# KudanLimited/cuda-bundle-adjustment

Measured on AMD Instinct MI355X. Metric: ba_edge_iterations_per_sec, higher is better.
Workload: dtype f64

## Files before the change

cuda-bundle-adjustment_amd/csrc/host/c_api.cpp:

```cpp
#include <cmath>
#include <cstring>
#include <deque>
#include <memory>
#include <unordered_map>

#include "../../../include/cugo_hip.h"
#include "../../include/cuda_graph_optimisation.h"
#include "../../include/icp_types.h"
#include "../kernels/kernels.h"
#include "chol_solver.h"
#include "engine.h"
#include "hip_util.h"
#include "rccl_comm.h"
#include "schur_plan.h"

using namespace cugo_host;

namespace
{
template <typename F>
int guarded(F&& f)
{
    try
    {
// ... 349 lines not shown
    return CUGO_OK;
}

int cugo_chol_plan_array(cugo_chol* s, const char* name, const int32_t** out)
{
    const CholPlan& P = s->plan;
    const std::string n(name);
    const std::vector<int32_t>* v = nullptr;
#define CUGO_PLAN_FIELD(f) \
    if (n == #f)           \
    v = &P.f
    CUGO_PLAN_FIELD(perm);
    CUGO_PLAN_FIELD(super_ptr);
    CUGO_PLAN_FIELD(rows_ptr);
    CUGO_PLAN_FIELD(rows);
    CUGO_PLAN_FIELD(sparent);
    CUGO_PLAN_FIELD(child_ptr);
    CUGO_PLAN_FIELD(child);
    CUGO_PLAN_FIELD(rel_ptr);
    CUGO_PLAN_FIELD(rel);
    CUGO_PLAN_FIELD(ncb);
    CUGO_PLAN_FIELD(nb);
    CUGO_PLAN_FIELD(col0);
    CUGO_PLAN_FIELD(col_front);
    CUGO_PLAN_FIELD(stage_task_ptr);
    CUGO_PLAN_FIELD(task_ptr);
    CUGO_PLAN_FIELD(task_fronts);
    CUGO_PLAN_FIELD(blk_front);
    CUGO_PLAN_FIELD(blk_row);
    CUGO_PLAN_FIELD(blk_col);
    CUGO_PLAN_FIELD(alias_of);
    CUGO_PLAN_FIELD(asm_map);
    CUGO_PLAN_FIELD(wl);
#undef CUGO_PLAN_FIELD
    if (n == "asm_info")
    {
        s->asm_info.assign(1, P.asm0);
        s->asm_info.push_back(P.nasm);
        for (int64_t o : P.asm_off)
            s->asm_info.push_back((int32_t)o);
        v = &s->asm_info;
    }
    if (n == "blk_trans")
        v = &s->trans32;
    if (n == "ea1")
        v = &s->ea1;
    if (!v)
    {
        set_last_error("cugo_chol_plan_array: unknown array " + n);
        return CUGO_ERR_INVALID;
    }
    *out = v->data();
    return (int)v->size();
}

int cugo_chol_plan_array64(cugo_chol* s, const char* name, const int64_t** out)
{
    const CholPlan& P = s->plan;
    const std::string n(name);
    const std::vector<int64_t>* v = n == "off" ? &P.off : n == "ldf" ? &P.ldf : n == "woff" ? &P.woff
                                  : n == "l21off" ? &P.l21off : nullptr;
    if (!v)
    {
        set_last_error("cugo_chol_plan_array64: unknown array " + n);
        return CUGO_ERR_INVALID;
    }
// ... 552 lines not shown
```

cuda-bundle-adjustment_amd/csrc/host/chol_solver.cpp:

```cpp
#include "chol_solver.h"

#include <cstdio>
#include <cstdlib>
#include <cstring>
#include <string>

using namespace cugo_host;

void cugo_chol::pack()
{
    const CholPlan& P = plan;
    pack32.clear(), pack64.clear();
    auto put32 = [this](const std::vector<int32_t>& v) {
        const size_t o = pack32.size();
        pack32.insert(pack32.end(), v.begin(), v.end());
        pack32.resize((pack32.size() + 3) & ~size_t(3));
        return o;
    };
    auto put64 = [this](const std::vector<int64_t>& v) {
        const size_t o = pack64.size();
        pack64.insert(pack64.end(), v.begin(), v.end());
        pack64.resize((pack64.size() + 1) & ~size_t(1));
        return o;
    };
// ... 53 lines not shown
        const int64_t q[4] = {P.off[f], P.ldf[f], P.woff[f], P.l21off[f]};
        std::memcpy(m + 8, q, sizeof q);
    }
    const size_t o_tmeta = put32(tmeta);
    std::vector<int32_t> fat(16 * (P.wl.size() / 3), 0);
    for (size_t i = 0; i < P.wl.size() / 3; i++)
    {
        int32_t* m = fat.data() + 16 * i;
        const int f = P.wl[3 * i];
        m[0] = f, m[1] = P.wl[3 * i + 1], m[2] = P.wl[3 * i + 2];
        if (f < 0 || f >= P.n_super)
            continue;
        m[3] = 6 * P.ncb[f], m[4] = 6 * (P.nb[f] - P.ncb[f]);
        m[5] = P.bw_np[f], m[6] = P.col0[f], m[7] = P.rows_ptr[f];
        const int64_t q[4] = {P.off[f], P.ldf[f], P.woff[f], P.l21off[f]};
        std::memcpy(m + 8, q, sizeof q);
        if ((int)i >= P.asm0 && (int)i < P.asm0 + P.nasm)
        {
            const int64_t nb = P.nb[f], mo = P.asm_off[f];
            m[5] = (int32_t)nb;
            std::memcpy(m + 6, &mo, sizeof mo);
            bool any = false;
            for (int64_t cb = m[1]; cb < m[2]; cb++)
            {
                any = any || P.asm_map[mo + cb] >= 0;
                const int64_t c0 = mo + nb + cb * nb - cb * (cb - 1) / 2;
                for (int64_t k = 0; k < nb - cb && !any; k++)
                    any = P.asm_map[c0 + k] >= 0;
            }
            m[4] = any ? 1 : 0;
        }
    }
    const size_t o_fat = put32(fat);
    const size_t o_asm_map = put32(P.asm_map);
    const size_t o_trans = pack32.size();
    pack32.resize(o_trans + (P.blk_trans.size() + 3) / 4 + 4, 0);
    if (!P.blk_trans.empty())
        std::memcpy(pack32.data() + o_trans, P.blk_trans.data(), P.blk_trans.size());
    const size_t o_asm_off = put64(P.asm_off);
    const size_t o_off = put64(P.off), o_woff = put64(P.woff), o_l21off = put64(P.l21off), o_ldf = put64(P.ldf);
    po = {o_ncb, o_nb, o_col0, o_alias, o_bwnp, o_lanp, o_rows_ptr, o_rows, o_child_ptr, o_child, o_rel_ptr, o_rel,
          o_task_ptr, o_task_fronts, o_blk_front, o_blk_row, o_blk_col, o_perm, o_col_front, o_wl, o_ea1, o_tmeta,
          o_fat, o_asm_map, o_trans, o_asm_off, o_off, o_woff, o_l21off, o_ldf};
}

void cugo_chol::upload(hipStream_t s)
{
    const CholPlan& P = plan;
    const size_t o_ncb = po[0], o_nb = po[1], o_col0 = po[2], o_alias = po[3], o_bwnp = po[4], o_lanp = po[5];
    const size_t o_rows_ptr = po[6], o_rows = po[7], o_child_ptr = po[8], o_child = po[9], o_rel_ptr = po[10];
    const size_t o_rel = po[11], o_task_ptr = po[12], o_task_fronts = po[13], o_blk_front = po[14], o_blk_row = po[15];
    const size_t o_blk_col = po[16], o_perm = po[17], o_col_front = po[18], o_wl = po[19], o_ea1 = po[20];
    const size_t o_tmeta = po[21], o_fat = po[22], o_asm_map = po[23], o_trans = po[24], o_asm_off = po[25];
    const size_t o_off = po[26], o_woff = po[27], o_l21off = po[28], o_ldf = po[29];
    d_pack32.upload(pack32, s), d_pack64.upload(pack64, s);
    d_fronts.resize((size_t)P.front_doubles + 16);
    d_fronts.zero(s);
    d_xnew.resize((size_t)6 * P.n + 16);
    d_junk.resize(64 * 1024);
    d_winv.resize((size_t)P.winv_doubles + 16);
    d_l21.resize((size_t)P.l21_doubles + 16);
    CUGO_HIP(hipStreamSynchronize(s));

    cugo_k::CholPlanDev& D = dev;
    D.n_fronts = P.n_super;
    const int32_t* b32 = d_pack32.data();
    const int64_t* b64 = d_pack64.data();
    D.ncb = b32 + o_ncb, D.nb = b32 + o_nb, D.off = b64 + o_off, D.col0 = b32 + o_col0;
    D.rows_ptr = b32 + o_rows_ptr, D.rows = b32 + o_rows;
    D.child_ptr = b32 + o_child_ptr, D.child = b32 + o_child;
    D.rel_ptr = b32 + o_rel_ptr, D.rel = b32 + o_rel;
    D.n_stages = P.n_stages;
    D.task_ptr = b32 + o_task_ptr, D.task_fronts = b32 + o_task_fronts, D.tmeta = b32 + o_tmeta;
    D.n_hsc_blocks = (int)P.blk_front.size();
    D.blk_front = b32 + o_blk_front, D.blk_row = b32 + o_blk_row;
    D.blk_col = b32 + o_blk_col, D.blk_trans = reinterpret_cast<const uint8_t*>(b32 + o_trans);
    D.n = P.n, D.perm = b32 + o_perm, D.col_front = b32 + o_col_front;
    D.junk = d_junk.data();
    D.woff = b64 + o_woff, D.winv = d_winv.data(), D.nc_max = P.nc_max;
    D.ea_lds = opt.ea_lds, D.panel16 = opt.panel16, D.ea_direct = opt.ea_direct;
#ifdef CUGO_DEBUG_HOOKS
    {
        const char* ka = std::getenv("CUGO_KERNEL_ACQUIRE");
        D.kernel_acquire = ka ? std::atoi(ka) & 7 : 0;
        const char* ed = std::getenv("CUGO_DEBUG_DELAY");
        D.dbg_delay = ed ? std::atoi(ed) : 0;
        const char* ez = std::getenv("CUGO_DEBUG_ZERO_LDS");
        D.zero_lds = ez ? std::atoi(ez) : 0, D.lds_doubles = 0;
        D.dbg_skip_wg = -1;
    }
#endif
    D.l21off = b64 + o_l21off, D.l21 = d_l21.data();
    D.ldf = b64 + o_ldf, D.alias_of = b32 + o_alias, D.bw_np = b32 + o_bwnp, D.la_np = b32 + o_lanp;
    d_wl_ptr = b32 + o_wl;
    D.wl_base = d_wl_ptr, D.fat = b32 + o_fat, D.ea1 = b32 + o_ea1;
    D.asm_map = b32 + o_asm_map, D.asm_off = b64 + o_asm_off;
    asm_fronts = opt.asm_fronts;
    lds_factor = cugo_k::chol_lds_factor_bytes(P.nc_max);
    lds_backward = cugo_k::chol_lds_backward_bytes(P.nc_max, P.ld_max);
}

void cugo_chol::analyze(int n, const int32_t* rowptr, const int32_t* colind)
{
    analyze_host(n, rowptr, colind);
    if (ctx)
        upload(ctx->stream);
}

void cugo_chol::analyze_host(int n, const int32_t* rowptr, const int32_t* colind)
{
    CholOptions copt = CholOptions::from_env();
    const bool own_forced = opt.own_subtrees == 1;
    if ((world > 1 || own_forced) && bcast && opt.own_subtrees != 0)
        copt.rank = rank, copt.world = world, copt.owned = true;
    chol_analyze(n, rowptr, colind, copt, plan);
    if (copt.owned && !own_forced && plan.flops < 1e9 * opt.own_min_gflop)
    {
        copt.rank = 0, copt.world = 1, copt.owned = false;
        chol_analyze(n, rowptr, colind, copt, plan);
    }
    lookahead = opt.lookahead;
    factored = false, si_ready = false, last_fail = nullptr;
    trans32.assign(plan.blk_trans.begin(), plan.blk_trans.end());
    pack();
    if (plan.nc_max > cugo_k::chol_max_pivot_cols() ||
        cugo_k::chol_lds_factor_bytes(plan.nc_max) > 160 * 1024 ||
        cugo_k::chol_lds_backward_bytes(plan.nc_max, plan.ld_max) > 160 * 1024)
        throw std::runtime_error("cugo: a front exceeds the LDS budget (nc=" +
                                 std::to_string(plan.nc_max) + ", ld=" + std::to_string(plan.ld_max) + ")");
// ... 143 lines not shown
    void keep_arrays(double* d_x)
    {
        if (!keep_on || c.dbg_calls > 16)
            return;
        const cugo_host::CholPlan& plan = c.plan;
        const size_t nf = (size_t)plan.front_doubles, nw = (size_t)plan.winv_doubles, nl = (size_t)plan.l21_doubles,
                     nx = (size_t)6 * plan.n;
        while (c.keep.size() < (size_t)c.dbg_calls)
            c.keep.emplace_back(new cugo_host::DevBuf<double>());
        auto& k = *c.keep[c.dbg_calls - 1];
        k.resize(nf + nw + nl + 2 * nx + 8);
        double* dst = k.data();
        const std::pair<const double*, size_t> parts[] = {{c.d_fronts.data(), nf}, {c.d_winv.data(), nw}, {c.d_l21.data(), nl},
                                                          {c.d_xnew.data(), nx}, {d_x, nx}};
        for (const auto& pr : parts)
        {
            if (pr.second)
                CUGO_HIP(hipMemcpyAsync(dst, pr.first, pr.second * sizeof(double), hipMemcpyDeviceToDevice, s));
            dst += pr.second;
        }
        g_last_kept = &c;
    }
};
#define CUGO_HOOK(expr) expr
#else
cugo_chol::~cugo_chol() {}
#define CUGO_HOOK(expr) ((void)0)
#endif

void cugo_chol::factor_solve(const double* d_Hsc, double lambda, const double* d_bsc, double* d_x,
                             int32_t* d_fail)
{
    hipStream_t s = ctx->stream;
    factored = true, last_fail = d_fail;
#ifdef CUGO_DEBUG_HOOKS
    cugo_chol_hooks hooks(*this);
#endif
#ifdef CUGO_STAMPS
    static const bool dbg = std::getenv("CUGO_DEBUG_STAMPS") != nullptr;
    static long long* d_stamps = nullptr;
    if (dbg && !d_stamps)
    {
        CUGO_HIP(hipMalloc(reinterpret_cast<void**>(&d_stamps), 64 * sizeof(long long)));
        CUGO_HIP(hipMemset(d_stamps, 0, 64 * sizeof(long long)));
        cugo_k::set_debug_stamps(d_stamps);
    }
#endif
    cugo_k::launch_chol_assemble(s, dev, d_fronts.data(), (size_t)plan.front_doubles, d_Hsc, lambda, d_bsc, d_fail,
                                 d_wl_ptr + 3L * plan.clr0, plan.nclr, asm_fronts ? d_wl_ptr + 3L * plan.asm0 : nullptr,
                                 plan.nasm);
    CUGO_HOOK(hooks.hash(11, d_fronts.data(), (size_t)plan.front_doubles));
    int pend0 = 0, npend = 0, pend_tile = 64;
    for (int st = 0; st < plan.n_stages; st++)
    {
        const int t0 = plan.stage_task_ptr[st], t1 = plan.stage_task_ptr[st + 1];
        if (plan.has_subtree_stage && st == 0)
            cugo_k::launch_chol_subtree_stage(s, dev, d_fronts.data(), t0, t1 - t0, lds_factor, d_fail);
        else if (lookahead)
        {
            cugo_k::launch_chol_potrf_la(s, dev, d_fronts.data(), t0, t1 - t0, d_wl_ptr + 3L * pend0, npend,
                                         pend_tile, d_fail);
            cugo_k::launch_chol_lead(s, dev, d_fronts.data(), d_wl_ptr + 3L * plan.lead_ptr[st],
                                     plan.lead_ptr[st + 1] - plan.lead_ptr[st], d_wl_ptr + 3L * plan.ea_ptr[st],
                                     plan.ea_ptr[st + 1] - plan.ea_ptr[st], d_wl_ptr + 3L * plan.eab_ptr[st],
                                     plan.eab_ptr[st + 1] - plan.eab_ptr[st]);
            pend0 = plan.sb_ptr[st], npend = plan.sb_ptr[st + 1] - plan.sb_ptr[st];
// ... 9 lines not shown
                plan.ea_ptr[st + 1] - plan.ea_ptr[st], plan.eab_ptr[st],
                plan.eab_ptr[st + 1] - plan.eab_ptr[st], plan.syrk_ptr[st],
                plan.syrk_ptr[st + 1] - plan.syrk_ptr[st], plan.stage_tile[st], lds_factor, d_fail, stale, stale_scratch);
            if (plan.stage_tile[st] == 0)
            {
                cugo_k::launch_chol_two_phase(s, dev, d_fronts.data(), d_wl_ptr + 3L * plan.trsm_ptr[st],
                                              plan.trsm_ptr[st + 1] - plan.trsm_ptr[st],
                                              d_wl_ptr + 3L * plan.syrk_ptr[st],
                                              plan.syrk_ptr[st + 1] - plan.syrk_ptr[st]);
                CUGO_HOOK(hooks.after_two_phase(st));
            }
        }
        CUGO_HOOK(hooks.after_level(st));
        bool grouped = false;
        for (size_t k = 0; k < plan.xu_front.size(); k++)
            if (plan.xu_stage[k] == st)
            {
                if (!grouped && bcast_group)
                    bcast_group(true), grouped = true;
                const int f = plan.xu_front[k];
                const int64_t ld = plan.ldf[f], c0 = 6LL * plan.ncb[f], c1 = 6LL * plan.nb[f];
                if (c1 > c0)
                    bcast(d_fronts.data() + plan.off[f] + c0 * ld + c0, (size_t)((c1 - 1 - c0) * ld + c1 + 1 - c0),
                          plan.xu_owner[k]);
            }
        if (grouped)
            bcast_group(false);
    }
    if (npend > 0)
        cugo_k::launch_chol_potrf_la(s, dev, d_fronts.data(), 0, 0, d_wl_ptr + 3L * pend0, npend, pend_tile, d_fail);
    CUGO_HOOK(hooks.hash(12, d_winv.data(), (size_t)plan.winv_doubles));
    CUGO_HOOK(hooks.hash(13, d_l21.data(), (size_t)plan.l21_doubles));
    CUGO_HOOK(hooks.hash(14, d_fronts.data(), (size_t)plan.front_doubles));
    for (int st = plan.n_stages - 1; st >= 0; st--)
    {
        const int t0 = plan.stage_task_ptr[st], t1 = plan.stage_task_ptr[st + 1];
        cugo_k::launch_chol_backward_stage(s, dev, d_fronts.data(), t0, t1 - t0, lds_backward, d_xnew.data(),
                                           d_x, d_wl_ptr + 3L * plan.bwg_ptr[st],
                                           plan.bwg_ptr[st + 1] - plan.bwg_ptr[st]);
        CUGO_HOOK(hooks.after_backward(st));
#ifdef CUGO_STAMPS
        if (dbg && st == plan.n_stages - 1)
        {
            CUGO_HIP(hipStreamSynchronize(s));
            CUGO_HIP(hipMemcpy(d_stamps + 48, d_stamps + 24, 8 * sizeof(long long), hipMemcpyDeviceToDevice));
        }
#endif
    }
    CUGO_HOOK(hooks.hash(15, d_xnew.data(), (size_t)6 * plan.n));
    if (!plan.xx_lo.empty())
    {
        if (bcast_group)
            bcast_group(true);
        for (size_t k = 0; k < plan.xx_lo.size(); k++)
            bcast(d_xnew.data() + 6LL * plan.xx_lo[k], (size_t)(6LL * (plan.xx_hi[k] - plan.xx_lo[k])), plan.xx_owner[k]);
        if (bcast_group)
            bcast_group(false);
        cugo_k::launch_chol_unpermute(s, dev, d_xnew.data(), d_x);
    }
    CUGO_HIP(hipGetLastError());
    CUGO_HOOK(hooks.keep_arrays(d_x));
#ifdef CUGO_STAMPS
    if (dbg)
    {
        long long h[64];
        CUGO_HIP(hipStreamSynchronize(s));
        CUGO_HIP(hipMemcpy(h, d_stamps, sizeof h, hipMemcpyDeviceToHost));
        static int calls = 0;
        if (++calls == 5)
            for (int k = 0; k < 7; k++)
            {
                std::printf("stamps kernel %d (nc=%lld):", k, h[k * 8 + 6]);
                for (int i = 1; i < 8; i++)
                    if (i != 6 && h[k * 8 + i])
                        std::printf(" [%d] +%lld", i, h[k * 8 + i] - h[k * 8]);
                std::printf("  (cycles since kernel start; last launch of the kernel)\n");
            }
    }
#endif
}

bool cugo_chol::selected_inverse(double* d_sigma)
{
    hipStream_t s = ctx->stream;
    int32_t h_fail = 0;
    CUGO_HIP(hipMemcpyAsync(&h_fail, last_fail, sizeof h_fail, hipMemcpyDeviceToHost, s));
    CUGO_HIP(hipStreamSynchronize(s));
    if (h_fail)
        return false;
    const CholPlan& P = plan;
    if (!si_ready)
    {
        std::vector<int64_t> sinfo(4 * (size_t)P.n_super + 4, 0);
        for (int f = 0; f < P.n_super; f++)
        {
            const int pa = P.sparent[f];
            if (pa < 0)
                continue;
            sinfo[4 * f] = P.off[pa], sinfo[4 * f + 1] = P.ldf[pa], sinfo[4 * f + 2] = P.rel_ptr[f];
            sinfo[4 * f + 3] = P.alias_of[pa] == f ? 0 : 1;
        }
        const int tile = cugo_k::selinv_row_tile();
        std::vector<int32_t> items;
        si_ptr.assign(P.n_stages + 1, 0);
        for (int st = 0; st < P.n_stages; st++)
        {
            si_ptr[st] = (int32_t)(items.size() / 2);
            if (!(P.has_subtree_stage && st == 0))
                for (int t = P.stage_task_ptr[st]; t < P.stage_task_ptr[st + 1]; t++)
                    for (int fi = P.task_ptr[t]; fi < P.task_ptr[t + 1]; fi++)
                    {
                        const int f = P.task_fronts[fi];
                        for (int r0 = 0; r0 < 6 * (P.nb[f] - P.ncb[f]); r0 += tile)
                            items.push_back(f), items.push_back(r0);
                    }
        }
        si_ptr[P.n_stages] = (int32_t)(items.size() / 2);
        items.resize(items.size() + 2, 0);
        d_sinfo.upload(sinfo, s);
        d_sitems.upload(items, s);
// ... 22 lines not shown
```

cuda-bundle-adjustment_amd/csrc/host/chol_solver.h:

```cpp
#pragma once
#include "../kernels/kernels.h"
#include "chol_symbolic.h"
#include "hip_util.h"
#include "options.h"

#include <array>
#include <functional>
#include <memory>

struct cugo_chol
{
    cugo_ctx* ctx = nullptr;
    bool analyzed = false;
    cugo_host::Options opt = cugo_host::Options::from_env();
    cugo_host::CholPlan plan;
    std::vector<int32_t> trans32;
    std::vector<int32_t> asm_info;
    std::vector<int32_t> ea1;
    cugo_k::CholPlanDev dev{};
    size_t lds_factor = 0, lds_backward = 0;
    bool lookahead = false;
    bool asm_fronts = true;

    std::vector<int32_t> pack32;
    std::vector<int64_t> pack64;
    std::array<size_t, 30> po{};
    cugo_host::DevBuf<int32_t> d_pack32;
    cugo_host::DevBuf<int64_t> d_pack64;
    const int32_t* d_wl_ptr = nullptr;
    cugo_host::DevBuf<double> d_fronts, d_xnew, d_junk, d_winv, d_l21;

    int rank = 0, world = 1;
    std::function<void(double*, size_t, int)> bcast;
    std::function<void(bool)> bcast_group;
    ~cugo_chol();
#ifdef CUGO_DEBUG_HOOKS
    unsigned long long* dbg_hash = nullptr;
    int dbg_calls = 0;
    std::vector<std::unique_ptr<cugo_host::DevBuf<double>>> keep;
    cugo_host::DevBuf<double> dbg_scratch;
    void dump_kept(const char* dir);
    void dump_slot(int call, const char* path);
#endif
    bool own_subtrees() const { return bcast && plan.owned; }

    const int32_t* last_fail = nullptr;
    bool factored = false;
    bool si_ready = false;
    cugo_host::DevBuf<double> d_sig;
    cugo_host::DevBuf<int64_t> d_sinfo;
    cugo_host::DevBuf<int32_t> d_sitems;
    std::vector<int32_t> si_ptr;
    bool selected_inverse(double* d_sigma);

    void analyze(int n, const int32_t* rowptr, const int32_t* colind);
    void analyze_host(int n, const int32_t* rowptr, const int32_t* colind);
    void pack();
    void upload(hipStream_t s);
    void factor_solve(const double* d_Hsc, double lambda, const double* d_bsc, double* d_x,
                      int32_t* d_fail);
};

#ifdef CUGO_DEBUG_HOOKS
// ... 5 lines not shown
```

cuda-bundle-adjustment_amd/csrc/host/chol_symbolic.cpp:

```cpp
#include "chol_symbolic.h"

#include <algorithm>
#include <atomic>
#include <chrono>
#include <cstdio>
#include <cstdlib>
#include <functional>
#include <numeric>
#include <stdexcept>
#include <thread>
#include <tuple>

namespace cugo_host
{

CholOptions CholOptions::from_env()
{
    CholOptions o;
    if (const char* s = std::getenv("CUGO_ND_LEAF"))
        o.nd_leaf = std::max(1, std::atoi(s));
    if (const char* s = std::getenv("CUGO_MAX_SUPER_COLS"))
        o.max_super_cols = std::max(1, std::atoi(s));
    if (const char* s = std::getenv("CUGO_ZERO_FRAC"))
        o.zero_frac = std::atof(s);
// ... 1420 lines not shown
                P.asm_off[f] = (int64_t)P.asm_map.size();
                P.asm_map.resize(P.asm_map.size() + nb + nb * (nb + 1) / 2, -1);
                for (int cb = 0; cb < nb; cb += 2)
                {
                    P.wl.push_back(f), P.wl.push_back(cb), P.wl.push_back((int)std::min<int64_t>(nb, cb + 2));
                    P.nasm++;
                }
            }
        for (int f = 0; f < ns; f++)
            if (P.asm_off[root[f]] >= 0)
                for (int c = 0; c < P.ncb[f]; c++)
                    P.asm_map[P.asm_off[root[f]] + shift[f] + c] = P.col0[f] + c;
        for (size_t k = 0; k < P.blk_front.size(); k++)
        {
            const int f = P.blk_front[k], o = root[f];
            if (P.asm_off[o] < 0)
                continue;
            const int64_t nb = P.nb[o], rb = P.blk_row[k] + shift[f], cb = P.blk_col[k] + shift[f];
            if (rb < cb || rb >= nb)
                throw std::runtime_error("cugo: an Hsc block outside the lower triangle of its front");
            int32_t& e = P.asm_map[P.asm_off[o] + nb + cb * nb - cb * (cb - 1) / 2 + (rb - cb)];
            if (e != -1)
                throw std::runtime_error("cugo: two Hsc blocks in one front position");
            e = 2 * (int32_t)k + (rb != cb && P.blk_trans[k] ? 1 : 0);
        }
    }
    for (auto& v : P.lead_ptr)
        v += (int)P.wl.size() / 3;
    P.wl.insert(P.wl.end(), lead.begin(), lead.end());
    for (auto& v : P.sb_ptr)
        v += (int)P.wl.size() / 3;
    P.wl.insert(P.wl.end(), sb.begin(), sb.end());
    lap("8 work items");
}

}
```

cuda-bundle-adjustment_amd/csrc/host/chol_symbolic.h:

```cpp
#pragma once
#include <cstdint>
#include <vector>

namespace cugo_host
{

struct CholOptions
{
    int nd_refine = 1;
    int nd_leaf = 96;
    int max_super_cols = 16;
    double zero_frac = 0.35;
    int target_tasks = 1024;
    bool alias_chains = true;
    int min_subtree_tasks = 1 << 30;
    int max_front_cols = 16;
    int two_phase_min_tiles = 260;
    bool xcd_affinity = true;
    int tile32_max_tiles = 64;
    int rank = 0, world = 1;
    bool owned = false;
    static CholOptions from_env();
};

// ... 7 lines not shown
    std::vector<int32_t> rows_ptr, rows;
    std::vector<int32_t> sparent;
    std::vector<int32_t> child_ptr, child;
    std::vector<int32_t> rel_ptr, rel;
    std::vector<int32_t> ncb, nb, col0;
    std::vector<int64_t> off;
    int64_t front_doubles = 0;
    std::vector<int64_t> ldf;
    std::vector<int32_t> alias_of;
    int n_aliased = 0;
    std::vector<int64_t> woff;
    int64_t winv_doubles = 0;
    std::vector<int64_t> l21off;
    int64_t l21_doubles = 0;
    std::vector<int32_t> col_front;

    int n_stages = 0;
    int sum_slots = 0;
    int nd_refined = 0;
    std::vector<int32_t> stage_task_ptr;
    std::vector<int32_t> task_ptr, task_fronts;
    bool has_subtree_stage = false;
    std::vector<int32_t> wl;
    std::vector<int32_t> ea_ptr, eab_ptr, syrk_ptr, bwg_ptr;
    int clr0 = 0, nclr = 0;
    int asm0 = 0, nasm = 0;
    std::vector<int32_t> asm_map;
    std::vector<int64_t> asm_off;
    std::vector<int32_t> la_np;
    std::vector<int32_t> lead_ptr, sb_ptr;
    std::vector<int32_t> stage_tile;
    std::vector<int32_t> trsm_ptr;
    std::vector<int32_t> bw_np;
    int nc_max = 6;

    std::vector<int32_t> owner;
    std::vector<int32_t> xu_front, xu_stage, xu_owner;
    std::vector<int32_t> xx_lo, xx_hi, xx_owner;
    double rank_flops = 0, top_flops = 0;
    bool owned = false;
    int64_t xs_seg = 0, xs_top = 0;
    std::vector<int64_t> xs_off;

    std::vector<int32_t> blk_front, blk_row, blk_col;
    std::vector<uint8_t> blk_trans;

    long ld_max = 1;
    double nnzL = 0;
    double flops = 0;
    double up_potrf_flops = 0, up_trsm_flops = 0, up_syrk_flops = 0, up_ea_bytes = 0, backward_bytes = 0;
};

void chol_analyze(int n, const int32_t* rowptr, const int32_t* colind, const CholOptions& opt,
                  CholPlan& plan);

}
```

cuda-bundle-adjustment_amd/csrc/host/options.h:

```cpp
#pragma once
#include <cstdlib>

namespace cugo_host
{

struct Options
{
    int hsc_mfma = 1;
    bool hsc_xcd = true;
    bool hsc_rows = false, hsc_strip = false, schur_plan = false;
    bool fuse_t = true;
    bool pose_schur = true;
    bool float32 = false;
    bool speculate = true, trial_event = true, trial_poll = true;
    bool trial_from_build = true;
    bool profile = false;
    bool init_timing = false;
    bool structure_reuse = true;
    bool flatten_reuse = true;
    bool async_structure = true;
    bool host_structure = false;
    bool upload_thread = true;
    int own_subtrees = -1;
    double own_min_gflop = 3.0;
    bool lookahead = false;
    bool ea_lds = true, panel16 = true, asm_fronts = true;
    bool ea_direct = true;
    bool reduce_scatter = true;

    static Options from_env()
    {
        Options o;
        auto flag = [](const char* name) { return std::getenv(name) != nullptr; };
        auto off = [](const char* name) {
            const char* e = std::getenv(name);
            return e && e[0] == '0';
        };
        auto on = [](const char* name) {
            const char* e = std::getenv(name);
            return e && e[0] == '1';
        };
        if (const char* e = std::getenv("CUGO_HSC_MFMA"))
            o.hsc_mfma = e[0] == '0' ? 0 : e[0] == '2' ? 2 : 1;
        o.hsc_xcd = !off("CUGO_HSC_XCD");
        o.schur_plan = flag("CUGO_SCHUR_PLAN");
        o.hsc_rows = on("CUGO_HSC_ROWS"), o.hsc_strip = on("CUGO_HSC_STRIP");
        o.fuse_t = !off("CUGO_FUSE_T");
        o.pose_schur = !off("CUGO_POSE_SCHUR");
        o.float32 = on("CUGO_FLOAT32");
        o.speculate = !off("CUGO_SPECULATE"), o.trial_event = !off("CUGO_TRIAL_EVENT"), o.trial_poll = !off("CUGO_TRIAL_POLL");
        o.trial_from_build = !off("CUGO_TRIAL_FROM_BUILD");
        o.profile = flag("CUGO_PROFILE");
        o.init_timing = flag("CUGO_INIT_TIMING");
        o.structure_reuse = !flag("CUGO_NO_STRUCTURE_REUSE");
        o.flatten_reuse = !flag("CUGO_NO_FLATTEN_REUSE");
        o.async_structure = !off("CUGO_ASYNC_STRUCTURE");
        o.host_structure = flag("CUGO_HOST_STRUCTURE");
        o.upload_thread = !off("CUGO_UPLOAD_THREAD");
        if (const char* e = std::getenv("CUGO_OWN_SUBTREES"))
            o.own_subtrees = e[0] == '1' ? 1 : e[0] == '0' ? 0 : -1;
        if (const char* e = std::getenv("CUGO_OWN_MIN_GFLOP"))
            o.own_min_gflop = std::atof(e);
        if (const char* e = std::getenv("CUGO_LOOKAHEAD"))
            o.lookahead = std::atoi(e) != 0;
        o.ea_lds = !off("CUGO_EA_LDS"), o.panel16 = !off("CUGO_PANEL16"), o.asm_fronts = !off("CUGO_ASM_FRONTS");
        o.ea_direct = !off("CUGO_EA_DIRECT");
        o.reduce_scatter = !off("CUGO_REDUCE_SCATTER");
        return o;
    }
};

}
```

cuda-bundle-adjustment_amd/csrc/kernels/chol_kernels.hip:

```cpp
#include <algorithm>
#include <cstdio>

#include "kernels.h"

namespace
{

constexpr int CBS = 256;
constexpr double PIVOT_TOL = 1e-14;
constexpr int TR = 64;
constexpr int NC_MAX = 96;
constexpr int LLD = NC_MAX + 17;
constexpr int PW = 6;

using cugo_k::CholPlanDev;
typedef double double4_t __attribute__((ext_vector_type(4)));

__device__ __forceinline__ void assemble_scatter(const CholPlanDev& p, double* __restrict__ fronts,
                                                 const double* __restrict__ Hsc, double lambda,
                                                 const double* __restrict__ bsc, int32_t* __restrict__ fail, int nblk,
                                                 int bid)
{
    if (bid >= nblk)
    {
// ... 2155 lines not shown

__global__ __launch_bounds__(BIG) void k_backward_stage(CholPlanDev p,
                                                        const double* __restrict__ fronts,
                                                        int task0, int ntasks,
                                                        const int32_t* __restrict__ wl_gemv,
                                                        double* __restrict__ xnew,
                                                        double* __restrict__ xout)
{
#ifdef CUGO_DEBUG_HOOKS
    if (p.dbg_skip_wg == (int)blockIdx.x)
        return;
#endif
    kernel_acquire(p);
    extern __shared__ double lds[];
    dbg_fill_lds(p, lds);
    if ((int)blockIdx.x >= ntasks)
    {
        dev_backward_ahead(p, p.fat + 16 * ((int)((wl_gemv - p.wl_base) / 3) + ((int)blockIdx.x - ntasks)), lds, xnew);
        kernel_release(p);
        return;
    }
    stamp(3, 0);
    const int task = task0 + blockIdx.x;
    const int32_t* tm = p.tmeta + cugo_k::TMETA * task;
    if (tm[0] == 1)
        dev_backward(p, fronts, front_view(tm), lds, xnew, xout, tm + 20);
    else
        for (int fi = p.task_ptr[task + 1] - 1; fi >= p.task_ptr[task]; fi--)
            dev_backward(p, fronts, front_view(p, p.task_fronts[fi]), lds, xnew, xout);
    stamp(3, 7);
    kernel_release(p);
}

__global__ __launch_bounds__(CBS) void k_unpermute(CholPlanDev p, const double* __restrict__ xnew, double* __restrict__ xout)
{
    const int i = blockIdx.x * CBS + threadIdx.x;
    if (i < 6 * p.n)
        xout[6L * p.perm[i / 6] + i % 6] = xnew[i];
}

__global__ __launch_bounds__(CBS) void k_xs_pack(const int64_t* __restrict__ off, int B, int n,
                                                 const double* __restrict__ sys, double* __restrict__ xbuf)
{
    const long i = (long)blockIdx.x * CBS + threadIdx.x;
    const long nH = 36L * B;
    if (i >= nH + 6L * n)
        return;
    const long dst = i < nH ? off[i / 36] + i % 36 : off[B + (i - nH) / 6] + (i - nH) % 6;
    xbuf[dst] = sys[i];
}
__global__ __launch_bounds__(CBS) void k_xs_unpack(const int64_t* __restrict__ off, int B, int n,
                                                   const double* __restrict__ xbuf, double* __restrict__ sys,
                                                   long lo, long hi, long top0)
{
    const long i = (long)blockIdx.x * CBS + threadIdx.x;
    const long nH = 36L * B;
    if (i >= nH + 6L * n)
        return;
    const long o = i < nH ? off[i / 36] : off[B + (i - nH) / 6];
    if ((o >= lo && o < hi) || o >= top0)
        sys[i] = xbuf[o + (i < nH ? i % 36 : (i - nH) % 6)];
}

__global__ void k_flag_to_double(int32_t* __restrict__ flag)
{
    const int v = *flag;
// ... 51 lines not shown
        g_skip.dump = std::fopen(dump_path, "w");
}
void chol_dbg_skip_end()
{
    if (g_skip.dump)
        std::fclose(g_skip.dump), g_skip.dump = nullptr;
    g_skip.target_launch = -1;
}
#endif

size_t chol_lds_factor_bytes(int nc_max)
{
    (void)nc_max;
    const size_t trsm = (size_t)NC_MAX * LLD + NC_MAX + std::max((size_t)(NC_MAX >> 4) * (16 * 17), (size_t)NC_MAX * PSTB);
    const size_t syrk = (size_t)syrk_lds();
    return (std::max(trsm, syrk) + 8) * sizeof(double);
}
size_t chol_lds_potrf_bytes()
{
    return std::max((size_t)NC_MAX * LLD + NC_MAX + (NC_MAX >> 4) * (16 * 17) + 8, (size_t)p16::LDS_DOUBLES + 8) *
           sizeof(double);
}
int chol_max_pivot_cols() { return NC_MAX; }
size_t chol_lds_backward_bytes(int nc_max, long ld_max)
{
    const size_t ncp = (size_t)((nc_max + 15) & ~15);
    return (ncp + (size_t)ld_max + 8) * sizeof(double);
}

void set_debug_stamps(long long* d_buf)
{
#ifdef CUGO_STAMPS
    (void)hipMemcpyToSymbol(HIP_SYMBOL(g_stamps), &d_buf, sizeof(d_buf));
#else
    (void)d_buf;
#endif
}

void launch_chol_assemble(hipStream_t s, const CholPlanDev& p, double* d_fronts,
                          size_t front_doubles, const double* d_Hsc, double lambda,
                          const double* d_bsc, int32_t* d_fail, const int32_t* d_clear_items, int nclear,
                          const int32_t* d_asm_items, int nasm)
{
    if (d_asm_items && nasm > 0)
    {
        const long n = 36L * p.n_hsc_blocks;
        const int nblk = (int)((n + CBS - 1) / CBS), nrhs = std::max(1, (6 * p.n + CBS - 1) / CBS);
        CUGO_LAUNCH(k_assemble_fronts, dim3(nasm + nblk + nrhs), dim3(CBS), 0, s, p, d_fronts, d_Hsc, lambda, d_bsc,
                    d_fail, (int)((d_asm_items - p.wl_base) / 3), nasm, nblk);
        return;
    }
    if (nclear > 0)
        CUGO_LAUNCH(k_clear_fronts, dim3(nclear), dim3(CBS), 0, s, p, d_fronts, d_clear_items);
    else
        (void)hipMemsetAsync(d_fronts, 0, front_doubles * sizeof(double), s);
    const long n = 36L * p.n_hsc_blocks;
    const int nblk = (int)((n + CBS - 1) / CBS), nrhs = std::max(1, (6 * p.n + CBS - 1) / CBS);
    CUGO_LAUNCH(k_assemble_blocks, dim3(nblk + nrhs), dim3(CBS), 0, s, p, d_fronts, d_Hsc, lambda, d_bsc, d_fail,
                nblk);
}

void launch_chol_subtree_stage(hipStream_t s, const CholPlanDev& p, double* d_fronts, int task0,
                               int ntasks, size_t lds_bytes, int32_t* d_fail)
{
    if (ntasks <= 0)
        return;
// ... 107 lines not shown

void launch_xs_pack(hipStream_t s, const int64_t* d_off, int B, int n, const double* d_sys, double* d_xbuf)
{
    const long total = 36L * B + 6L * n;
    if (total > 0)
        CUGO_LAUNCH(k_xs_pack, dim3((unsigned)((total + CBS - 1) / CBS)), dim3(CBS), 0, s, d_off, B, n, d_sys, d_xbuf);
}
void launch_xs_unpack(hipStream_t s, const int64_t* d_off, int B, int n, const double* d_xbuf, double* d_sys, long lo,
                      long hi, long top0)
{
    const long total = 36L * B + 6L * n;
    if (total > 0)
        CUGO_LAUNCH(k_xs_unpack, dim3((unsigned)((total + CBS - 1) / CBS)), dim3(CBS), 0, s, d_off, B, n, d_xbuf, d_sys,
                    lo, hi, top0);
}

void launch_chol_unpermute(hipStream_t s, const CholPlanDev& p, const double* d_xnew, double* d_x)
{
    if (p.n > 0)
        CUGO_LAUNCH(k_unpermute, dim3((6 * p.n + CBS - 1) / CBS), dim3(CBS), 0, s, p, d_xnew, d_x);
}

void launch_chol_backward_stage(hipStream_t s, const CholPlanDev& p, double* d_fronts, int task0,
                                int ntasks, size_t lds_bytes, double* d_xnew, double* d_x,
                                const int32_t* d_wl_gemv, int ngemv)
{
    if (ntasks <= 0)
        return;
    ensure_lds(reinterpret_cast<const void*>(k_backward_stage), lds_bytes);
    CUGO_LAUNCH(k_backward_stage, dim3(ntasks + ngemv), dim3(BIG), lds_bytes, s, with_lds(p, lds_bytes, "k_backward_stage", ntasks + ngemv, ntasks), d_fronts, task0,
                       ntasks, d_wl_gemv, d_xnew, d_x);
}

}
```

cuda-bundle-adjustment_amd/csrc/kernels/kernels.h:

```cpp
#pragma once
#include <hip/hip_runtime.h>
#include <stddef.h>
#include <stdint.h>

#include "../../../include/cugo_hip.h"

namespace cugo_k
{

struct LaunchHook
{
    virtual void begin(const char* kernel, hipStream_t s) = 0;
    virtual void end(const char* kernel, hipStream_t s) = 0;
    virtual ~LaunchHook() {}
};
void set_launch_hook(LaunchHook* h);
LaunchHook* launch_hook();
struct LaunchScope
{
    const char* name;
    hipStream_t s;
    LaunchHook* h;
    LaunchScope(const char* n, hipStream_t st) : name(n), s(st), h(launch_hook())
    {
// ... 97 lines not shown
    const int64_t* ldf;
    const int32_t* alias_of;
    const int32_t* bw_np;
    const int32_t* la_np;
    const int64_t* woff;
    double* winv;
    const int64_t* l21off;
    double* l21;
    int nc_max;
    int ea_lds;
    int panel16;
    int ea_direct;
#ifdef CUGO_DEBUG_HOOKS
    int kernel_acquire;
    int dbg_delay;
    int zero_lds;
    int lds_doubles;
    int dbg_skip_wg;
#endif
    const int32_t* col0;
    const int32_t* rows_ptr;
    const int32_t* rows;
    const int32_t* child_ptr;
    const int32_t* child;
    const int32_t* rel_ptr;
    const int32_t* rel;
    int n_stages;
    const int32_t* ea1;
    const int32_t* tmeta;
    const int32_t* asm_map;
    const int64_t* asm_off;
    const int32_t* wl_base;
    const int32_t* fat;
    const int32_t* task_ptr;
    const int32_t* task_fronts;
    int n_hsc_blocks;
    const int32_t* blk_front;
    const int32_t* blk_row;
    const int32_t* blk_col;
    const uint8_t* blk_trans;
    int n;
    const int32_t* perm;
    const int32_t* col_front;
    double* junk;
};

void launch_chol_assemble(hipStream_t s, const CholPlanDev& p, double* d_fronts, size_t front_doubles,
                          const double* d_Hsc, double lambda, const double* d_bsc, int32_t* d_fail,
                          const int32_t* d_clear_items, int nclear, const int32_t* d_asm_items = nullptr,
                          int nasm = 0);
void launch_chol_subtree_stage(hipStream_t s, const CholPlanDev& p, double* d_fronts, int task0,
                               int ntasks, size_t lds_bytes, int32_t* d_fail);
void launch_chol_upper_stage(hipStream_t s, const CholPlanDev& p, double* d_fronts, int task0,
                             int ntasks, const int32_t* d_wl, int eap0, int neap, int ea0, int nea,
                             int sy0, int nsy, int tile, size_t lds_bytes, int32_t* d_fail,
                             double* dbg_line = nullptr, double* dbg_scratch = nullptr);
#ifdef CUGO_DEBUG_HOOKS
void launch_swap16(hipStream_t s, double* line, double* scratch);
#endif
void launch_chol_two_phase(hipStream_t s, const CholPlanDev& p, double* d_fronts, const int32_t* d_trsm, int ntrsm,
                           const int32_t* d_syrk, int nsyrk);
void launch_chol_potrf_la(hipStream_t s, const CholPlanDev& p, double* d_fronts, int task0, int ntasks,
                          const int32_t* d_tiles, int ntiles, int tile, int32_t* d_fail);
void launch_chol_lead(hipStream_t s, const CholPlanDev& p, double* d_fronts, const int32_t* d_lead,
                      int nlead, const int32_t* d_eap, int neap, const int32_t* d_eab, int neab);
void launch_chol_backward_stage(hipStream_t s, const CholPlanDev& p, double* d_fronts, int task0,
                                int ntasks, size_t lds_bytes, double* d_xnew, double* d_x,
                                const int32_t* d_wl_gemv, int ngemv);
#ifdef CUGO_DEBUG_HOOKS
void launch_nop(hipStream_t s);
void chol_dbg_skip_begin(int target_launch, int target_wg, const char* dump_path);
void chol_dbg_skip_end();
void launch_hash_words(hipStream_t s, const void* p, size_t n_words, unsigned long long* out);
#endif
void launch_flag_to_double(hipStream_t s, int32_t* d_flag);
void launch_chol_unpermute(hipStream_t s, const CholPlanDev& p, const double* d_xnew, double* d_x);
void launch_xs_pack(hipStream_t s, const int64_t* d_off, int B, int n, const double* d_sys, double* d_xbuf);
void launch_xs_unpack(hipStream_t s, const int64_t* d_off, int B, int n, const double* d_xbuf, double* d_sys, long lo,
                      long hi, long top0);
void set_debug_stamps(long long* d_buf);
size_t chol_lds_factor_bytes(int nc_max);
size_t chol_lds_backward_bytes(int nc_max, long ld_max);
int chol_max_pivot_cols();

void launch_selinv_rows(hipStream_t s, const CholPlanDev& p, const double* d_fronts, double* d_sig,
                        const int64_t* d_sinfo, const int32_t* d_items, int nitems);
void launch_selinv_jj(hipStream_t s, const CholPlanDev& p, const double* d_fronts, double* d_sig, int task0,
                      int ntasks);
void launch_selinv_subtree(hipStream_t s, const CholPlanDev& p, const double* d_fronts, double* d_sig,
                           const int64_t* d_sinfo, int task0, int ntasks);
void launch_selinv_gather(hipStream_t s, const CholPlanDev& p, const double* d_sig, double* d_out);
int selinv_row_tile();
void launch_cov_pose_diag(hipStream_t s, int P, const int32_t* d_rowptr, const double* d_sigma, double* d_out);
void launch_lm_covariance(hipStream_t s, int L, const int32_t* d_lm_ptr, const int32_t* d_e_pose,
                          const uint8_t* d_flags, const double* d_Hll, const double* d_Hpl, const int32_t* d_rowptr,
                          const int32_t* d_colind, const double* d_sigma, double* d_out, int32_t* d_fail);

}
```

Measured before the change: 618.3 million.

## Replace staged backward substitution with single-launch dependency-chained kernel

Replaces the per-stage loop of backward-substitution launches with one kernel in which each workgroup takes a ticket in schedule order. Each workgroup spins on per-front done flags (epoch-tagged) for the boundary fronts it reads before consuming their solved values. This removes the many stage launches and the barriers between stages on the backward solve. In exchange it relies on ticket ordering for forward progress, adds a spin timeout with an error path, and needs new segment metadata built during symbolic analysis.

```diff
diff --git a/cuda-bundle-adjustment_amd/csrc/host/c_api.cpp b/cuda-bundle-adjustment_amd/csrc/host/c_api.cpp
--- a/cuda-bundle-adjustment_amd/csrc/host/c_api.cpp
+++ b/cuda-bundle-adjustment_amd/csrc/host/c_api.cpp
@@ -405,6 +405,9 @@
     CUGO_PLAN_FIELD(alias_of);
     CUGO_PLAN_FIELD(asm_map);
     CUGO_PLAN_FIELD(wl);
+    CUGO_PLAN_FIELD(bc_front);
+    CUGO_PLAN_FIELD(bc_seg_ptr);
+    CUGO_PLAN_FIELD(bc_seg);
 #undef CUGO_PLAN_FIELD
     if (n == "asm_info")
     {
diff --git a/cuda-bundle-adjustment_amd/csrc/host/chol_solver.cpp b/cuda-bundle-adjustment_amd/csrc/host/chol_solver.cpp
--- a/cuda-bundle-adjustment_amd/csrc/host/chol_solver.cpp
+++ b/cuda-bundle-adjustment_amd/csrc/host/chol_solver.cpp
@@ -109,6 +109,19 @@
         }
     }
     const size_t o_fat = put32(fat);
+    std::vector<int32_t> bc_rec(cugo_k::BC_REC * P.bc_front.size(), 0), bc_seg(4 * (P.bc_seg.size() / 3) + 4, 0);
+    for (size_t t = 0; t < P.bc_front.size(); t++)
+    {
+        int32_t* m = bc_rec.data() + cugo_k::BC_REC * t;
+        const int f = P.bc_front[t];
+        m[0] = f, m[1] = P.ncb[f], m[2] = P.nb[f], m[3] = P.col0[f], m[4] = P.rows_ptr[f];
+        m[5] = P.bc_seg_ptr[f], m[6] = P.bc_seg_ptr[f + 1] - P.bc_seg_ptr[f];
+        const int64_t q[4] = {P.woff[f], P.l21off[f], P.off[f], P.ldf[f]};
+        std::memcpy(m + 8, q, sizeof q);
+    }
+    for (size_t k = 0; k < P.bc_seg.size() / 3; k++)
+        std::memcpy(bc_seg.data() + 4 * k, P.bc_seg.data() + 3 * k, 3 * sizeof(int32_t));
+    const size_t o_bc_rec = put32(bc_rec), o_bc_seg = put32(bc_seg);
     const size_t o_asm_map = put32(P.asm_map);
     const size_t o_trans = pack32.size();
     pack32.resize(o_trans + (P.blk_trans.size() + 3) / 4 + 4, 0);
@@ -118,7 +131,7 @@
     const size_t o_off = put64(P.off), o_woff = put64(P.woff), o_l21off = put64(P.l21off), o_ldf = put64(P.ldf);
     po = {o_ncb, o_nb, o_col0, o_alias, o_bwnp, o_lanp, o_rows_ptr, o_rows, o_child_ptr, o_child, o_rel_ptr, o_rel,
           o_task_ptr, o_task_fronts, o_blk_front, o_blk_row, o_blk_col, o_perm, o_col_front, o_wl, o_ea1, o_tmeta,
-          o_fat, o_asm_map, o_trans, o_asm_off, o_off, o_woff, o_l21off, o_ldf};
+          o_fat, o_asm_map, o_trans, o_asm_off, o_off, o_woff, o_l21off, o_ldf, o_bc_rec, o_bc_seg};
 }
 
 void cugo_chol::upload(hipStream_t s)
@@ -130,6 +143,7 @@
     const size_t o_blk_col = po[16], o_perm = po[17], o_col_front = po[18], o_wl = po[19], o_ea1 = po[20];
     const size_t o_tmeta = po[21], o_fat = po[22], o_asm_map = po[23], o_trans = po[24], o_asm_off = po[25];
     const size_t o_off = po[26], o_woff = po[27], o_l21off = po[28], o_ldf = po[29];
+    const size_t o_bc_rec = po[30], o_bc_seg = po[31];
     d_pack32.upload(pack32, s), d_pack64.upload(pack64, s);
     d_fronts.resize((size_t)P.front_doubles + 16);
     d_fronts.zero(s);
@@ -137,6 +151,15 @@
     d_junk.resize(64 * 1024);
     d_winv.resize((size_t)P.winv_doubles + 16);
     d_l21.resize((size_t)P.l21_doubles + 16);
+    bw_chain = opt.bw_chain && !opt.lookahead && !P.has_subtree_stage && !P.bc_front.empty();
+    if (bw_chain)
+    {
+        d_bc_state.resize((size_t)cugo_k::BC_DONE + P.n_super);
+        d_bc_state.zero(s);
+        h_bc_error.resize(1);
+        h_bc_error[0] = 0;
+        bc_base = 0, bc_epoch = 0;
+    }
     CUGO_HIP(hipStreamSynchronize(s));
 
     cugo_k::CholPlanDev& D = dev;
@@ -172,6 +195,7 @@
     d_wl_ptr = b32 + o_wl;
     D.wl_base = d_wl_ptr, D.fat = b32 + o_fat, D.ea1 = b32 + o_ea1;
     D.asm_map = b32 + o_asm_map, D.asm_off = b64 + o_asm_off;
+    D.bc_rec = b32 + o_bc_rec, D.bc_seg = b32 + o_bc_seg;
     asm_fronts = opt.asm_fronts;
     lds_factor = cugo_k::chol_lds_factor_bytes(P.nc_max);
     lds_backward = cugo_k::chol_lds_backward_bytes(P.nc_max, P.ld_max);
@@ -381,6 +405,7 @@
                              int32_t* d_fail)
 {
     hipStream_t s = ctx->stream;
+    check_chain_error();
     factored = true, last_fail = d_fail;
 #ifdef CUGO_DEBUG_HOOKS
     cugo_chol_hooks hooks(*this);
@@ -456,7 +481,52 @@
     CUGO_HOOK(hooks.hash(12, d_winv.data(), (size_t)plan.winv_doubles));
     CUGO_HOOK(hooks.hash(13, d_l21.data(), (size_t)plan.l21_doubles));
     CUGO_HOOK(hooks.hash(14, d_fronts.data(), (size_t)plan.front_doubles));
-    for (int st = plan.n_stages - 1; st >= 0; st--)
+    if (bw_chain)
+    {
+        const int nf = (int)plan.bc_front.size();
+        if (++bc_epoch == 0)
+            bc_epoch = 1;
+        cugo_k::launch_chol_backward_chain(s, dev, d_fronts.data(), nf, d_xnew.data(), d_x, d_bc_state.data(), bc_base,
+                                           bc_epoch, d_fail, h_bc_error.data());
+        bc_base += (uint32_t)nf;
+#ifdef CUGO_STAMPS
+        if (dbg)
+        {
+            static int chain_calls = 0;
+            static long long* d_cs = nullptr;
+            if (++chain_calls == 4)
+            {
+                CUGO_HIP(hipMalloc(reinterpret_cast<void**>(&d_cs), 3 * sizeof(long long) * (size_t)nf));
+                CUGO_HIP(hipMemset(d_cs, 0, 3 * sizeof(long long) * (size_t)nf));
+                cugo_k::set_chain_stamps(d_cs);
+            }
+            if (chain_calls == 5)
+            {
+                std::vector<long long> h(3 * (size_t)nf);
+                std::vector<int> ticket(plan.n_super, -1);
+                for (int t = 0; t < nf; t++)
+                    ticket[plan.bc_front[t]] = t;
+                CUGO_HIP(hipStreamSynchronize(s));
+                CUGO_HIP(hipMemcpy(h.data(), d_cs, h.size() * sizeof(long long), hipMemcpyDeviceToHost));
+                cugo_k::set_chain_stamps(nullptr);
+                long long first = h[0], last = 0;
+                for (int t = 0; t < nf; t++)
+                    first = std::min(first, h[3 * t]), last = std::max(last, h[3 * t + 2]);
+                std::printf("chain stamps: %d fronts, first start to last done %lld ticks (10 ns)\n", nf, last - first);
+                for (int f = plan.bc_front[nf - 1]; f >= 0; f = plan.sparent[f])
+                {
+                    const int t = ticket[f], pa = plan.sparent[f];
+                    std::printf("  front %d ticket %d ncb %d rows %d: start +%lld", f, t, plan.ncb[f], plan.nb[f] - plan.ncb[f],
+                                h[3 * t] - first);
+                    if (pa >= 0)
+                        std::printf(" wait %lld work %lld", h[3 * t + 1] - h[3 * ticket[pa] + 2], h[3 * t + 2] - h[3 * t + 1]);
+                    std::printf(" done +%lld\n", h[3 * t + 2] - first);
+                }
+            }
+        }
+#endif
+    }
+    for (int st = plan.n_stages - 1; st >= 0 && !bw_chain; st--)
     {
         const int t0 = plan.stage_task_ptr[st], t1 = plan.stage_task_ptr[st + 1];
         cugo_k::launch_chol_backward_stage(s, dev, d_fronts.data(), t0, t1 - t0, lds_backward, d_xnew.data(),
@@ -504,12 +574,19 @@
 #endif
 }
 
+void cugo_chol::check_chain_error()
+{
+    if (bw_chain && h_bc_error.data() && *static_cast<volatile uint32_t*>(h_bc_error.data()) != 0)
+        throw std::runtime_error("cugo: the backward substitution gave up waiting for a front (k_backward_chain)");
+}
+
 bool cugo_chol::selected_inverse(double* d_sigma)
 {
     hipStream_t s = ctx->stream;
     int32_t h_fail = 0;
     CUGO_HIP(hipMemcpyAsync(&h_fail, last_fail, sizeof h_fail, hipMemcpyDeviceToHost, s));
     CUGO_HIP(hipStreamSynchronize(s));
+    check_chain_error();
     if (h_fail)
         return false;
     const CholPlan& P = plan;
diff --git a/cuda-bundle-adjustment_amd/csrc/host/chol_solver.h b/cuda-bundle-adjustment_amd/csrc/host/chol_solver.h
--- a/cuda-bundle-adjustment_amd/csrc/host/chol_solver.h
+++ b/cuda-bundle-adjustment_amd/csrc/host/chol_solver.h
@@ -24,11 +24,16 @@
 
     std::vector<int32_t> pack32;
     std::vector<int64_t> pack64;
-    std::array<size_t, 30> po{};
+    std::array<size_t, 32> po{};
     cugo_host::DevBuf<int32_t> d_pack32;
     cugo_host::DevBuf<int64_t> d_pack64;
     const int32_t* d_wl_ptr = nullptr;
     cugo_host::DevBuf<double> d_fronts, d_xnew, d_junk, d_winv, d_l21;
+    bool bw_chain = false;
+    cugo_host::DevBuf<uint32_t> d_bc_state;
+    cugo_host::PinnedBuf<uint32_t> h_bc_error;
+    uint32_t bc_base = 0, bc_epoch = 0;
+    void check_chain_error();
 
     int rank = 0, world = 1;
     std::function<void(double*, size_t, int)> bcast;
diff --git a/cuda-bundle-adjustment_amd/csrc/host/chol_symbolic.cpp b/cuda-bundle-adjustment_amd/csrc/host/chol_symbolic.cpp
--- a/cuda-bundle-adjustment_amd/csrc/host/chol_symbolic.cpp
+++ b/cuda-bundle-adjustment_amd/csrc/host/chol_symbolic.cpp
@@ -1476,6 +1476,33 @@
         v += (int)P.wl.size() / 3;
     P.wl.insert(P.wl.end(), sb.begin(), sb.end());
     lap("8 work items");
+    P.bc_front.clear(), P.bc_seg.clear();
+    P.bc_seg_ptr.assign(ns + 1, 0);
+    std::vector<int32_t> ticket(ns, -1);
+    for (int st = P.n_stages - 1; st >= 0; st--)
+        for (int t = P.stage_task_ptr[st]; t < P.stage_task_ptr[st + 1]; t++)
+            for (int fi = P.task_ptr[t + 1] - 1; fi >= P.task_ptr[t]; fi--)
+            {
+                ticket[P.task_fronts[fi]] = (int32_t)P.bc_front.size();
+                P.bc_front.push_back(P.task_fronts[fi]);
+            }
+    for (int f = 0; f < ns; f++)
+    {
+        const int r0 = P.rows_ptr[f], r1 = P.rows_ptr[f + 1];
+        for (int k = r0; k < r1;)
+        {
+            const int a = P.col_front[P.rows[k]];
+            int e = k + 1;
+            while (e < r1 && e - k < 16 && P.col_front[P.rows[e]] == a)
+                e++;
+            if (ticket[f] >= 0 && !(ticket[a] >= 0 && ticket[a] < ticket[f]))
+                throw std::runtime_error("cugo: a boundary row of a front belongs to a front scheduled after it");
+            P.bc_seg.push_back(a), P.bc_seg.push_back(k - r0), P.bc_seg.push_back(e - k);
+            k = e;
+        }
+        P.bc_seg_ptr[f + 1] = (int32_t)(P.bc_seg.size() / 3);
+    }
+    lap("9 backward chain");
 }
 
 }
diff --git a/cuda-bundle-adjustment_amd/csrc/host/chol_symbolic.h b/cuda-bundle-adjustment_amd/csrc/host/chol_symbolic.h
--- a/cuda-bundle-adjustment_amd/csrc/host/chol_symbolic.h
+++ b/cuda-bundle-adjustment_amd/csrc/host/chol_symbolic.h
@@ -63,6 +63,7 @@
     std::vector<int32_t> stage_tile;
     std::vector<int32_t> trsm_ptr;
     std::vector<int32_t> bw_np;
+    std::vector<int32_t> bc_front, bc_seg_ptr, bc_seg;
     int nc_max = 6;
 
     std::vector<int32_t> owner;
diff --git a/cuda-bundle-adjustment_amd/csrc/host/options.h b/cuda-bundle-adjustment_amd/csrc/host/options.h
--- a/cuda-bundle-adjustment_amd/csrc/host/options.h
+++ b/cuda-bundle-adjustment_amd/csrc/host/options.h
@@ -26,6 +26,7 @@
     bool lookahead = false;
     bool ea_lds = true, panel16 = true, asm_fronts = true;
     bool ea_direct = true;
+    bool bw_chain = true;
     bool reduce_scatter = true;
 
     static Options from_env()
@@ -65,6 +66,7 @@
             o.lookahead = std::atoi(e) != 0;
         o.ea_lds = !off("CUGO_EA_LDS"), o.panel16 = !off("CUGO_PANEL16"), o.asm_fronts = !off("CUGO_ASM_FRONTS");
         o.ea_direct = !off("CUGO_EA_DIRECT");
+        o.bw_chain = !off("CUGO_BW_CHAIN");
         o.reduce_scatter = !off("CUGO_REDUCE_SCATTER");
         return o;
     }
diff --git a/cuda-bundle-adjustment_amd/csrc/kernels/chol_kernels.hip b/cuda-bundle-adjustment_amd/csrc/kernels/chol_kernels.hip
--- a/cuda-bundle-adjustment_amd/csrc/kernels/chol_kernels.hip
+++ b/cuda-bundle-adjustment_amd/csrc/kernels/chol_kernels.hip
@@ -2211,6 +2211,164 @@
     kernel_release(p);
 }
 
+typedef __attribute__((address_space(1))) unsigned int gu32;
+typedef __attribute__((address_space(1))) unsigned long long gu64;
+#ifdef CUGO_STAMPS
+__device__ long long* g_bc_stamps = nullptr;
+__device__ __forceinline__ void bc_stamp(int ticket, int slot)
+{
+    if (g_bc_stamps && threadIdx.x == 0)
+        g_bc_stamps[3 * ticket + slot] = (long long)__builtin_amdgcn_s_memrealtime();
+}
+#else
+__device__ __forceinline__ void bc_stamp(int, int) {}
+#endif
+constexpr unsigned long long BW_SPIN_TICKS = 25000000ULL;
+
+__device__ __forceinline__ void bw_wait(gu32* word, unsigned epoch, gu32* st, int32_t* fail, unsigned* h_error)
+{
+    if (__hip_atomic_load(word, __ATOMIC_RELAXED, __HIP_MEMORY_SCOPE_AGENT) == epoch)
+        return;
+    const unsigned long long t0 = __builtin_amdgcn_s_memrealtime();
+    for (;;)
+    {
+        __builtin_amdgcn_s_sleep(1);
+        if (__hip_atomic_load(word, __ATOMIC_RELAXED, __HIP_MEMORY_SCOPE_AGENT) == epoch)
+            return;
+        if (__hip_atomic_load(st + cugo_k::BC_ABORT, __ATOMIC_RELAXED, __HIP_MEMORY_SCOPE_AGENT) != 0)
+            return;
+        if (__builtin_amdgcn_s_memrealtime() - t0 > BW_SPIN_TICKS)
+        {
+            __hip_atomic_store(st + cugo_k::BC_ABORT, 1u, __ATOMIC_RELAXED, __HIP_MEMORY_SCOPE_AGENT);
+            __hip_atomic_store(st + cugo_k::BC_ERROR, 1u, __ATOMIC_RELAXED, __HIP_MEMORY_SCOPE_AGENT);
+            __hip_atomic_store(fail, 1, __ATOMIC_RELAXED, __HIP_MEMORY_SCOPE_AGENT);
+            __hip_atomic_store(h_error, 1u, __ATOMIC_RELAXED, __HIP_MEMORY_SCOPE_SYSTEM);
+            return;
+        }
+    }
+}
+
+__global__ __launch_bounds__(BIG) void k_backward_chain(CholPlanDev p, const double* __restrict__ fronts,
+                                                        double* xnew, double* __restrict__ xout, unsigned* state,
+                                                        unsigned ticket_base, unsigned epoch, int32_t* fail,
+                                                        unsigned* h_error)
+{
+    kernel_acquire(p);
+    extern __shared__ double lds[];
+    dbg_fill_lds(p, lds);
+    gu32* st = (gu32*)state;
+    double* vs = lds;
+    int* tk = reinterpret_cast<int*>(lds + NC_MAX);
+    if (threadIdx.x == 0)
+        *tk = (int)(__hip_atomic_fetch_add(st + cugo_k::BC_HEAD, 1u, __ATOMIC_RELAXED, __HIP_MEMORY_SCOPE_AGENT) - ticket_base);
+    __syncthreads();
+    const int t = __builtin_amdgcn_readfirstlane(*tk);
+    if (t < 0 || t >= (int)gridDim.x)
+        return;
+#ifdef CUGO_DEBUG_HOOKS
+    const bool skip = p.dbg_skip_wg == t;
+#else
+    const bool skip = false;
+#endif
+    bc_stamp(t, 0);
+    const int32_t* rc = p.bc_rec + cugo_k::BC_REC * t;
+    const int f = rc[0], ncb = rc[1], nb = rc[2], c0 = rc[3], nseg = rc[6];
+    const int32_t* rows = p.rows + rc[4];
+    const int32_t* sg = p.bc_seg + 4 * rc[5];
+    const long* r64 = reinterpret_cast<const long*>(rc + 8);
+    const long l21o = r64[1], ld = r64[3];
+    const int ncs = 6 * ncb, nrs = 6 * (nb - ncb), ncp = pad16(ncs);
+    const double* L = l21o >= 0 ? p.l21 + l21o : fronts + r64[2] + ncs;
+    const long ldl = l21o >= 0 ? nrs + 1 : ld;
+    const double* Wg = p.winv + r64[0];
+    const int g = threadIdx.x >> 3, l8 = threadIdx.x & 7;
+    const bool colok = g < ncs;
+    const int j = min(g, ncs - 1);
+    const double* col = L + (long)j * ldl;
+    const double* wcol = Wg + (long)j * ncp;
+    const int jb = j / 6, comp = j - 6 * jb;
+    double wv[12];
+    const int k0 = (j & ~15) + 2 * l8;
+#pragma unroll
+    for (int u = 0; u < 6; u++)
+    {
+        const double2 v = *reinterpret_cast<const double2*>(wcol + min(k0 + 16 * u, ncp - 2));
+        wv[2 * u] = v.x, wv[2 * u + 1] = v.y;
+    }
+    const double y = col[nrs];
+    const int pj = p.perm[c0 + jb];
+    for (int jj = ncs + threadIdx.x; jj < ncp; jj += blockDim.x)
+        vs[jj] = 0.0;
+    gu64* xg = (gu64*)xnew;
+    double s = 0;
+    for (int q = nseg - 1; q >= 0; q--)
+    {
+        const int a = sg[4 * q], rb = sg[4 * q + 1], n6 = 6 * sg[4 * q + 2];
+        double b[12];
+        int xi[6];
+#pragma unroll
+        for (int u = 0; u < 6; u++)
+        {
+            const int i = min(2 * l8 + 16 * u, n6 - 2);
+            const double2 v = *reinterpret_cast<const double2*>(col + (6 * rb + i));
+            b[2 * u] = v.x, b[2 * u + 1] = v.y;
+            xi[u] = 6 * rows[rb + i / 6] + i % 6;
+        }
+#ifdef CUGO_DEBUG_HOOKS
+        if (p.dbg_delay == 31 && (t & 1) && q == nseg - 1)
+            dbg_sleep();
+#endif
+        if (threadIdx.x < 64)
+            bw_wait(st + cugo_k::BC_DONE + a, epoch, st, fail, h_error);
+        TILE_SYNC();
+        if (q == 0)
+            bc_stamp(t, 1);
+        __builtin_amdgcn_fence(__ATOMIC_ACQUIRE, "wavefront");
+        double x[12];
+#pragma unroll
+        for (int u = 0; u < 6; u++)
+        {
+            x[2 * u] = __longlong_as_double((long long)__hip_atomic_load(xg + xi[u], __ATOMIC_RELAXED, __HIP_MEMORY_SCOPE_AGENT));
+            x[2 * u + 1] = __longlong_as_double((long long)__hip_atomic_load(xg + xi[u] + 1, __ATOMIC_RELAXED, __HIP_MEMORY_SCOPE_AGENT));
+        }
+#pragma unroll
+        for (int u = 0; u < 12; u++)
+            s += (2 * l8 + 16 * (u >> 1) < n6) ? b[u] * x[u] : 0.0;
+    }
+#pragma unroll
+    for (int off = 4; off > 0; off >>= 1)
+        s += __shfl_xor(s, off, 8);
+    if (l8 == 0 && colok)
+        vs[j] = y - s;
+    TILE_SYNC();
+    double xj = 0;
+#pragma unroll
+    for (int u = 0; u < 12; u++)
+    {
+        const int k = k0 + 16 * (u >> 1) + (u & 1);
+        xj += (k < ncp) ? wv[u] * vs[k] : 0.0;
+    }
+#pragma unroll
+    for (int off = 4; off > 0; off >>= 1)
+        xj += __shfl_xor(xj, off, 8);
+    if (l8 == 0 && colok && !skip)
+    {
+        __hip_atomic_store(xg + (6L * (c0 + jb) + comp), (unsigned long long)__double_as_longlong(xj), __ATOMIC_RELAXED,
+                           __HIP_MEMORY_SCOPE_AGENT);
+        xout[6L * pj + comp] = xj;
+    }
+    asm volatile("s_waitcnt vmcnt(0)" ::: "memory");
+#ifdef CUGO_DEBUG_HOOKS
+    if (p.dbg_delay == 31 && (t & 1))
+        dbg_sleep();
+#endif
+    __syncthreads();
+    bc_stamp(t, 2);
+    if (threadIdx.x == 0)
+        __hip_atomic_store(st + cugo_k::BC_DONE + f, epoch, __ATOMIC_RELAXED, __HIP_MEMORY_SCOPE_AGENT);
+    kernel_release(p);
+}
+
 __global__ __launch_bounds__(CBS) void k_unpermute(CholPlanDev p, const double* __restrict__ xnew, double* __restrict__ xout)
 {
     const int i = blockIdx.x * CBS + threadIdx.x;
@@ -2328,6 +2486,14 @@
 {
 #ifdef CUGO_STAMPS
     (void)hipMemcpyToSymbol(HIP_SYMBOL(g_stamps), &d_buf, sizeof(d_buf));
+#else
+    (void)d_buf;
+#endif
+}
+void set_chain_stamps(long long* d_buf)
+{
+#ifdef CUGO_STAMPS
+    (void)hipMemcpyToSymbol(HIP_SYMBOL(g_bc_stamps), &d_buf, sizeof(d_buf));
 #else
     (void)d_buf;
 #endif
@@ -2501,4 +2667,16 @@
                        ntasks, d_wl_gemv, d_xnew, d_x);
 }
 
-}
+void launch_chol_backward_chain(hipStream_t s, const CholPlanDev& p, double* d_fronts, int nfronts, double* d_xnew,
+                                double* d_x, uint32_t* d_state, uint32_t ticket_base, uint32_t epoch, int32_t* d_fail,
+                                uint32_t* h_error)
+{
+    if (nfronts <= 0)
+        return;
+    const size_t lds_bytes = 96 * 1024;
+    ensure_lds(reinterpret_cast<const void*>(k_backward_chain), lds_bytes);
+    CUGO_LAUNCH(k_backward_chain, dim3(nfronts), dim3(BIG), lds_bytes, s, with_lds(p, lds_bytes, "k_backward_chain", nfronts),
+                d_fronts, d_xnew, d_x, d_state, ticket_base, epoch, d_fail, h_error);
+}
+
+}
diff --git a/cuda-bundle-adjustment_amd/csrc/kernels/kernels.h b/cuda-bundle-adjustment_amd/csrc/kernels/kernels.h
--- a/cuda-bundle-adjustment_amd/csrc/kernels/kernels.h
+++ b/cuda-bundle-adjustment_amd/csrc/kernels/kernels.h
@@ -153,6 +153,8 @@
     const int64_t* asm_off;
     const int32_t* wl_base;
     const int32_t* fat;
+    const int32_t* bc_rec;
+    const int32_t* bc_seg;
     const int32_t* task_ptr;
     const int32_t* task_fronts;
     int n_hsc_blocks;
@@ -188,6 +190,10 @@
 void launch_chol_backward_stage(hipStream_t s, const CholPlanDev& p, double* d_fronts, int task0,
                                 int ntasks, size_t lds_bytes, double* d_xnew, double* d_x,
                                 const int32_t* d_wl_gemv, int ngemv);
+constexpr int BC_REC = 16, BC_HEAD = 0, BC_ABORT = 32, BC_ERROR = 33, BC_DONE = 64;
+void launch_chol_backward_chain(hipStream_t s, const CholPlanDev& p, double* d_fronts, int nfronts, double* d_xnew,
+                                double* d_x, uint32_t* d_state, uint32_t ticket_base, uint32_t epoch, int32_t* d_fail,
+                                uint32_t* h_error);
 #ifdef CUGO_DEBUG_HOOKS
 void launch_nop(hipStream_t s);
 void chol_dbg_skip_begin(int target_launch, int target_wg, const char* dump_path);
@@ -200,6 +206,7 @@
 void launch_xs_unpack(hipStream_t s, const int64_t* d_off, int B, int n, const double* d_xbuf, double* d_sys, long lo,
                       long hi, long top0);
 void set_debug_stamps(long long* d_buf);
+void set_chain_stamps(long long* d_buf);
 size_t chol_lds_factor_bytes(int nc_max);
 size_t chol_lds_backward_bytes(int nc_max, long ld_max);
 int chol_max_pivot_cols();
```

After: 639.7 million, median of 6. +3.5%, better.
